# XiaRho/CMDA

Hardware: AMD Instinct MI355X
Metric: training images/sec (512x512 image+event, MiT-B5) (higher is better)
Workload: dtype bf16

## Files before the change

cmda_amd/csrc/gemm.hip:

```cpp
#include "gemm_kernels.h"

namespace {

template <typename T>
int launch_dtype(GemmParams& p, void* stream) {
  const long zb = (long)p.batch * p.batch2;
  auto blocks = [&](int bm, int bn) { return (long)((p.M + bm - 1) / bm) * ((p.N + bn - 1) / bn) * zb; };
  constexpr int BK = 8 * Num<T>::kChunk;
  const int nkt = (p.K + BK - 1) / BK;
  int tile;
  if (p.atomic && p.splits <= 0) {
    tile = 2;
    if (p.M > 64 && p.N > 64) {
      if (sizeof(T) == 2 && p.M >= 256 && p.N >= 256 && p.A.conv != 1 && (blocks(256, 256) >= 32 || (blocks(256, 256) >= 4 && nkt >= 1024)))
        tile = 3;
      else if (blocks(128, 128) >= 64 || (blocks(128, 128) >= 16 && nkt >= 1024)) tile = 0;
      else if (blocks(128, 64) >= 48 && nkt >= 256) tile = 1;
    }
    const long b = tile == 3 ? blocks(256, 256) : tile == 0 ? blocks(128, 128) : tile == 1 ? blocks(128, 64) : blocks(64, 64);
    long s = ((p.B.conv == 1 ? 1024 : 512) + b - 1) / b;
    s = std::min<long>(s, std::max(1, nkt / 8));
    const long out_bytes = (long)p.M * p.N * 4 * zb;
    s = std::min<long>(s, std::max<long>(16, (32L << 20) / std::max<long>(out_bytes, 1)));
    if (tile == 3 && b * s < 256) s = std::min<long>((256 + b - 1) / b, std::max(1, nkt / 8));
    s = std::min<long>(s, 128);
    s = std::min<long>(s, std::max<long>(1, 65535 / std::max<long>(zb, 1)));
    s = std::max<long>(1, s);
    {
      const long slots = 256L * (tile == 3 ? 1 : tile == 0 ? 2 : tile == 1 ? 3 : 4);
      double best = 1e30;
      for (long c = 1; c <= s; ++c) best = std::min(best, (double)((b * c + slots - 1) / slots) / (double)c);
      for (long c = 1; c <= s; ++c)
        if ((double)((b * c + slots - 1) / slots) / (double)c <= best * 1.05) {
          s = c;
          break;
        }
    }
    p.splits = (int)s;
  } else {
    if (p.splits <= 0) p.splits = 1;
    const long sp = p.splits;
    if (sizeof(T) == 2 && p.N >= 256 && p.K >= 256 && (blocks(256, 256) * sp >= 1024 || (blocks(256, 256) * sp >= 200 && p.K >= 2048))) tile = 3;
    else if (sizeof(T) == 2 && (p.N & 255) == 0 && p.K <= 1024 && blocks(256, 256) * sp >= 256 && !p.a_kstrided && !p.b_kstrided && p.A.conv != 1 &&
             p.B.conv != 1 && !p.res && !p.rowscale && p.beta == 0.f && !p.out_f32 && !p.atomic && p.c_patch_ow == 0)
      tile = 3;
    else if (p.N > 64 && (p.N & 127) > 0 && (p.N & 127) <= 64 && blocks(128, 64) * sp >= 2048) tile = 1;
    else if (p.N > 64 && blocks(128, 128) * sp >= 256) tile = 0;
    else if (blocks(128, 64) * sp >= 2048) tile = 1;
    else tile = 2;
    if (tile != 3 && blocks(128, 128) * sp < 1024 && p.M > 64 && p.N > 64) {
      const double nk = (double)nkt;
      const double cost0 = (double)((blocks(128, 128) * sp + 511) / 512) * (4.0 + 0.9 * nk);
      const bool lean = sizeof(T) == 2 && cmda_gemm_lean_ok_(p, 2);
      const double cost1 = (double)((blocks(128, 64) * sp + 767) / 768) * (lean ? 1.5 + 0.45 * nk : 3.0 + 0.75 * nk);
      const double cost2 = (double)((blocks(64, 64) * sp + 1023) / 1024) * (lean ? 1.2 + 0.3 * nk : 2.5 + 0.6 * nk);
      tile = cost0 <= cost1 && cost0 <= cost2 ? 0 : cost1 <= cost2 ? 1 : 2;
    }
  }
  if ((p.tile_hint & 15) >= 1 && (p.tile_hint & 15) <= 4 && p.tile_hint > 0) tile = (p.tile_hint & 15) - 1;
  if constexpr (sizeof(T) == 2) {
    const bool no_glds = p.tile_hint < 0;
    auto dma_ok = [&](const GemmView& v) {
      return v.vec_ok && (v.in_dil <= 1 || (v.conv == 1 && !v.reflect && &v == &p.A && !p.a_kstrided)) && v.R < (1L << 31) && v.Cc < (1L << 31) &&
             (!v.conv || (v.H < 32768 && v.W < 32768)) && (v.conv || (v.ld % 8) == 0) && (v.Cc % 8) == 0 &&
             (v.conv != 2 || ((v.KW * v.C) % 64 == 0 && v.KH == v.stride && v.KW == v.stride && v.pad == 0 && v.dil == 1 &&
                              v.H == v.OH * v.stride && v.W == v.OW * v.stride));
    };
    const bool ac = p.A.conv == 1, bc = p.B.conv == 1, aks = p.a_kstrided != 0, bks = p.b_kstrided != 0;
    const bool kind_ok = (!ac && !bc) || (ac && !bc && !aks && !bks) || (!ac && bc && aks && bks);
    const bool nt_plain = kind_ok && dma_ok(p.A) && dma_ok(p.B);
    if (p.colsum && !(nt_plain && !no_glds && aks)) return CMDA_ERR_UNSUPPORTED;
    if (nt_plain && !no_glds) {
      const bool pp_shape = (p.tile_hint > 0 && (p.tile_hint & 1024)) || (!ac && (p.K <= 1024 || bks));
      if (tile == 3 && pp_shape && !(p.tile_hint > 0 && (p.tile_hint & 512)) && !aks && !bc && !p.atomic && p.splits == 1 && !p.res &&
          !p.rowscale && p.beta == 0.f && !p.out_f32 && p.c_patch_ow == 0 && !p.colsum)
        return cmda_gemm_pp_(p, stream);
      if (tile == 3 && aks && bks && !ac && p.atomic && p.out_f32 && !(p.tile_hint > 0 && (p.tile_hint & 512)))
        return cmda_gemm_wg_(p, stream);
      if (tile == 3) return cmda_gemm_glds_t3_(p, stream);
      if (tile == 0) return cmda_gemm_glds_t0_(p, stream);
      if (!p.colstats && cmda_gemm_lean_ok_(p, tile)) {
        const long tl = tile == 1 ? blocks(128, 64) : blocks(64, 64);
        const int force = p.tile_hint > 0 ? ((p.tile_hint >> 4) & 15) : 0;
        const bool four_stage = force ? force == 4 : (tl <= 256L * (tile == 1 ? 1 : 2) && nkt >= 12);
        return cmda_gemm_lean_(p, tile, four_stage ? 1 : 0, stream);
      }
      if (tile == 1) return cmda_gemm_glds_t1_(p, stream);
      return cmda_gemm_glds_t2_(p, stream);
    }
  }
  if (p.colsum && !(p.dtype == CMDA_F32X3 && cmda_gemm_x3_lean_ok_(p))) return CMDA_ERR_UNSUPPORTED;
  return cmda_gemm_reg_(p, tile, stream);
}

}

extern "C" int cmda_gemm(const cmda_gemm_params_t* pp, void* stream) {
  if (!pp) return CMDA_ERR_SHAPE;
  GemmParams p = *pp;
  if (p.batch2 <= 0) p.batch2 = 1;
  if (p.M <= 0 || p.N <= 0 || p.batch <= 0) return CMDA_OK;
  if (p.K <= 0) return CMDA_ERR_SHAPE;
  if (p.atomic && !p.out_f32) return CMDA_ERR_UNSUPPORTED;
  if (p.splits > 1 && !p.atomic) return CMDA_ERR_UNSUPPORTED;
  if (p.atomic && (p.bias || p.act || p.res || p.rowscale)) return CMDA_ERR_UNSUPPORTED;
  if (p.colstats && (p.atomic || p.splits > 1 || p.act || p.rowscale || p.c_patch_ow > 0 || p.a_kstrided || p.batch != 1 || p.batch2 != 1 || (p.N & 3) ||
                     p.colstats_rows <= 0 || (p.colstats_rows & 255) || p.colsum))
    return CMDA_ERR_UNSUPPORTED;
  if (p.c_patch_ow > 0 && (p.atomic || p.res || p.batch != 1 || p.batch2 != 1 || p.c_patch_kh <= 0 || p.c_patch_kwci <= 0 ||
                           p.N != p.c_patch_kh * p.c_patch_kwci || p.M % p.c_patch_ow != 0 || (p.c_patch_kwci & 3)))
    return CMDA_ERR_UNSUPPORTED;
  if (p.dtype == CMDA_F32 || p.dtype == CMDA_F32X3) return launch_dtype<float>(p, stream);
  if (p.dtype == CMDA_BF16) return launch_dtype<bf16_t>(p, stream);
  return CMDA_ERR_DTYPE;
}

#ifdef CMDA_GEMM_TIMING
#include "gemm_t0.hip"
#include "gemm_t1.hip"
#include "gemm_t2.hip"
#include "gemm_t3.hip"
#include "gemm_reg.hip"
#include "gemm_reg_f32_t0.hip"
#include "gemm_reg_f32_t1.hip"
#include "gemm_reg_f32_t2.hip"
#include "gemm_reg_bf16_t0.hip"
#include "gemm_reg_bf16_t1.hip"
#include "gemm_reg_bf16_t2.hip"
extern "C" int cmda_debug_gemm_stamps(unsigned long long* host_out) {
  return hipMemcpyFromSymbol(host_out, HIP_SYMBOL(g_stamps), sizeof(unsigned long long) * 256 * 8) == hipSuccess ? 0 : -3;
}
#endif
```

cmda_amd/csrc/gemm_kernels.h:

```cpp
#pragma once
#include <cstdlib>
#include <type_traits>
#include "common.h"
#include "../../include/cmda_hip.h"

namespace {

typedef cmda_view_t GemmView;
typedef cmda_gemm_params_t GemmParams;

static __device__ __forceinline__ int reflect_idx(int i, int n) {
  if (i < 0) i = -i;
  if (i >= n) i = 2 * (n - 1) - i;
  return i;
}

static __device__ __forceinline__ long view_offset(const GemmView& v, long r, long c) {
  if (r >= v.R || c >= v.Cc) return -1;
  if (!v.conv) return r * v.ld + c;
  const int ohw = v.OH * v.OW;
  const int b = (int)(r / ohw);
  const int rem = (int)(r - (long)b * ohw);
  const int oh = rem / v.OW;
  const int ow = rem - oh * v.OW;
// ... 824 lines not shown
};

template <bool KS, bool CONV, bool FAST> struct DmaMode { static constexpr int value = !FAST ? 0 : (CONV ? (KS ? 3 : 2) : 1); };

template <int TM, int TN, bool AKS, bool BKS, bool ACONV, bool BCONV, int NW, int NSV, bool FAST = false>
static __device__ __forceinline__ void gemm_glds_body(const GemmParams& p, char* smem, int bt_raw, int ntile_raw, int z_raw, bool xcd_walk) {
  typedef bf16_t T;
  typedef GldsCfg<TM, TN, NW, NSV> Cfg;
  constexpr int WM = Cfg::WM, NTHR = Cfg::NTHR, BM = Cfg::BM, BN = Cfg::BN, BK = Cfg::BK, NS = Cfg::NS;
  constexpr int SZ_A = Cfg::SZ_A, SZ_B = Cfg::SZ_B, PITCH_C = Cfg::PITCH_C, EPI_ROWS = Cfg::EPI_ROWS;
  T* const sAbase = reinterpret_cast<T*>(smem);
  T* const sBbase = sAbase + NS * SZ_A;
  const int tid = threadIdx.x, lane = tid & 63, wid = tid >> 6;
  const int wm = wid >> 1, wn = wid & 1, g = lane >> 4, l15 = lane & 15;
  const int tiles_n = (p.N + BN - 1) / BN;
  const int ntile = ntile_raw;
  int bt = bt_raw;
  if (xcd_walk) {
    const int q = ntile / 8, rr = ntile % 8, xcd = bt % 8, loc = bt / 8;
    bt = (xcd < rr ? xcd * (q + 1) : rr * (q + 1) + (xcd - rr) * q) + loc;
  }
  long mt, nt;
  {
    constexpr int GM = NW == 8 ? 4 : 8;
    const int tiles_m = (int)((p.M + BM - 1) / BM);
    if (tiles_n >= 2 * GM && tiles_m >= GM && !(p.tile_hint > 0 && (p.tile_hint & 256))) {
      const int gsz = GM * tiles_n, gid = bt / gsz, first = gid * GM;
      const int gm = min(tiles_m - first, GM), r = bt - gid * gsz;
      mt = first + r % gm;
      nt = r / gm;
    } else {
      mt = bt / tiles_n;
      nt = bt % tiles_n;
    }
  }
  const long m0 = mt * BM;
  const long n0 = nt * BN;
  const int z = z_raw;
  const int bz = z / p.splits;
  const int split = z - bz * p.splits;
  const int batch = bz / p.batch2, batch2 = bz - batch * p.batch2;
  const int nkt = (p.K + BK - 1) / BK;
  const int kt_per = (nkt + p.splits - 1) / p.splits;
  const int kt0 = split * kt_per;
  const int kt1 = min(nkt, kt0 + kt_per);
  const T* baseA = reinterpret_cast<const T*>(p.A.ptr) + (long)batch * p.A.batch_stride + (long)batch2 * p.A.batch2_stride;
  const T* baseB = reinterpret_cast<const T*>(p.B.ptr) + (long)batch * p.B.batch_stride + (long)batch2 * p.B.batch2_stride;

  CMDA_STAMP(0);
  DmaSrc<AKS, BM, ACONV, NW, 0, 64, DmaMode<AKS, ACONV, FAST>::value> dA;
  DmaSrc<BKS, BN, BCONV, NW, 0, 64, DmaMode<BKS, BCONV, FAST>::value> dB;
  dA.init(p.A, baseA, wid, lane, m0, kt0);
  dB.init(p.B, baseB, wid, lane, n0, kt0);
  auto issue = [&](int stage, int kt) {
    char* la = reinterpret_cast<char*>(sAbase + stage * SZ_A) + wid * dA.J * 1024;
    char* lb = reinterpret_cast<char*>(sBbase + stage * SZ_B) + wid * dB.J * 1024;
    const bool fa = dA.cell_begin(kt, kt0, &p.A), fb = dB.cell_begin(kt, kt0, &p.B);
#pragma unroll
    for (int j = 0; j < dA.J; ++j) glds16(dA.get(p.A, baseA, j, kt, fa), la + j * 1024);
#pragma unroll
    for (int j = 0; j < dB.J; ++j) glds16(dB.get(p.B, baseB, j, kt, fb), lb + j * 1024);
  };

  f32x4 acc[TM][TN];
#pragma unroll
  for (int i = 0; i < TM; ++i)
#pragma unroll
    for (int j = 0; j < TN; ++j) acc[i][j] = f32x4{0.f, 0.f, 0.f, 0.f};

  const bool do_colsum = AKS && p.colsum != nullptr && n0 == 0;
  float bsum = 0.f;
  constexpr int LPT = DmaSrc<AKS, BM, ACONV, NW>::J + DmaSrc<BKS, BN, BCONV, NW>::J;
#pragma unroll
  for (int s = 0; s < NS - 1; ++s)
    if (kt0 + s < kt1) issue(s, kt0 + s);
  CMDA_STAMP(1);
  int st = 0;
  for (int kt = kt0; kt < kt1; ++kt) {
    if (kt + NS - 2 < kt1) pipe_barrier<(NS - 2) * LPT>();
    else pipe_barrier<0>();
    if (kt == kt0) CMDA_STAMP(2);
    {
      int sn = st + NS - 1;
      if (sn >= NS) sn -= NS;
      if (kt + NS - 1 < kt1) issue(sn, kt + NS - 1);
    }
    const T* sA = sAbase + st * SZ_A;
    const T* sB = sBbase + st * SZ_B;
    if constexpr (AKS) {
      if (do_colsum && tid < BM) {
#pragma unroll 8
        for (int k = 0; k < BK; ++k) bsum += bf2f(sA[k * BM + (((tid >> 3) ^ (k & 7)) << 3) + (tid & 7)]);
      }
    }
#pragma unroll
    for (int kk = 0; kk < 2; ++kk) {
      u16x8 fa[TM], fb[TN];
#pragma unroll
      for (int i = 0; i < TM; ++i) {
        const int mr = wm * 16 * TM + i * 16;
        if constexpr (!AKS) {
          const int row = mr + l15;
          fa[i] = *reinterpret_cast<const u16x8*>(&sA[row * BK + (((kk * 4 + g) ^ (row & 7)) << 3)]);
        } else {
          const int q = l15 >> 2, pp = l15 & 3;
          const int k0 = kk * 32 + 8 * g + q, k1 = k0 + 4;
          const int cidx = (mr >> 3) + (pp >> 1), half = (pp & 1) << 2;
          const u16x4 lo = lds_read_tr16(&sA[k0 * BM + ((cidx ^ (k0 & 7)) << 3) + half]);
          const u16x4 hi = lds_read_tr16(&sA[k1 * BM + ((cidx ^ (k1 & 7)) << 3) + half]);
          fa[i] = u16x8{lo[0], lo[1], lo[2], lo[3], hi[0], hi[1], hi[2], hi[3]};
        }
      }
#pragma unroll
      for (int j = 0; j < TN; ++j) {
        const int nr = wn * 16 * TN + j * 16;
        if constexpr (!BKS) {
          const int row = nr + l15;
          fb[j] = *reinterpret_cast<const u16x8*>(&sB[row * BK + (((kk * 4 + g) ^ (row & 7)) << 3)]);
        } else {
          const int q = l15 >> 2, pp = l15 & 3;
          const int k0 = kk * 32 + 8 * g + q, k1 = k0 + 4;
          const int cidx = (nr >> 3) + (pp >> 1), half = (pp & 1) << 2;
          const u16x4 lo = lds_read_tr16(&sB[k0 * BN + ((cidx ^ (k0 & 7)) << 3) + half]);
          const u16x4 hi = lds_read_tr16(&sB[k1 * BN + ((cidx ^ (k1 & 7)) << 3) + half]);
          fb[j] = u16x8{lo[0], lo[1], lo[2], lo[3], hi[0], hi[1], hi[2], hi[3]};
        }
      }
#pragma unroll
      for (int i = 0; i < TM; ++i)
#pragma unroll
        for (int j = 0; j < TN; ++j) acc[i][j] = mfma_bf16_16x16x32(fa[i], fb[j], acc[i][j]);
    }
    if (++st == NS) st = 0;
  }
  CMDA_STAMP(3);
  __syncthreads();

  if (kt0 >= kt1 && p.splits > 1) return;
  if constexpr (AKS) {
    if (do_colsum && tid < BM && m0 + tid < p.M) atomicAdd(p.colsum + m0 + tid, bsum);
  }
  const long cb = (long)batch * p.c_batch_stride + (long)batch2 * p.c_batch2_stride;
  const long rb_off = (long)batch * p.res_batch_stride + (long)batch2 * p.res_batch2_stride;
  if (p.atomic) {
#pragma unroll
    for (int i = 0; i < TM; ++i)
#pragma unroll
      for (int j = 0; j < TN; ++j) {
        const long n = n0 + wn * 16 * TN + j * 16 + l15;
#pragma unroll
        for (int r = 0; r < 4; ++r) {
          const long m = m0 + wm * 16 * TM + i * 16 + 4 * g + r;
          if (m < p.M && n < p.N) atomicAdd(reinterpret_cast<float*>(p.C) + cb + m * p.ldc + atomic_col(p, n), p.alpha * acc[i][j][r]);
        }
      }
    return;
  }
  float* sC = reinterpret_cast<float*>(smem);
  if constexpr (NW == 4) {
#pragma unroll
    for (int i = 0; i < TM; ++i)
#pragma unroll
      for (int j = 0; j < TN; ++j)
#pragma unroll
        for (int r = 0; r < 4; ++r)
          sC[(wm * 16 * TM + i * 16 + 4 * g + r) * PITCH_C + wn * 16 * TN + j * 16 + l15] = acc[i][j][r];
    __syncthreads();
    CMDA_STAMP(4);
    float cs[4] = {0.f, 0.f, 0.f, 0.f}, cq[4] = {0.f, 0.f, 0.f, 0.f};
    epilogue_store<T, BM, BN, PITCH_C, NTHR>(p, sC, m0, n0, cb, rb_off, tid, cs, cq);
    if (p.colstats) {
      __syncthreads();
      colstats_flush<BN, NTHR>(p, sC, m0, n0, tid, cs, cq);
    }
  } else {
    float cs[4] = {0.f, 0.f, 0.f, 0.f}, cq[4] = {0.f, 0.f, 0.f, 0.f};
    for (int wr = 0; wr < WM; ++wr) {
      if (wm == wr) {
#pragma unroll
        for (int i = 0; i < TM; ++i)
#pragma unroll
          for (int j = 0; j < TN; ++j)
#pragma unroll
            for (int r = 0; r < 4; ++r)
              sC[(i * 16 + 4 * g + r) * PITCH_C + wn * 16 * TN + j * 16 + l15] = acc[i][j][r];
      }
      __syncthreads();
      if (m0 + wr * EPI_ROWS < p.M)
        epilogue_store<T, EPI_ROWS, BN, PITCH_C, NTHR>(p, sC, m0 + wr * EPI_ROWS, n0, cb, rb_off, tid, cs, cq);
      __syncthreads();
    }
    if (p.colstats) colstats_flush<BN, NTHR>(p, sC, m0, n0, tid, cs, cq);
    CMDA_STAMP(4);
  }
  CMDA_STAMP(5);
}

template <int TM, int TN, bool AKS, bool BKS, bool ACONV, bool BCONV, int NW = 4, int NSV = 0, bool FAST = false>
__global__ __launch_bounds__(64 * NW, (GldsCfg<TM, TN, NW, NSV>::MIN_WAVES)) void gemm_glds_kernel(GemmParams p) {
  __shared__ __attribute__((aligned(1024))) char smem[GldsCfg<TM, TN, NW, NSV>::LDS_BYTES];
  gemm_glds_body<TM, TN, AKS, BKS, ACONV, BCONV, NW, NSV, FAST>(p, smem, blockIdx.x, gridDim.x, blockIdx.z, true);
}

template <int TM, int TN, bool AKS, bool BKS, bool ACONV, bool BCONV, int NW = 4, int NSV = 0, bool FAST = false>
__global__ __launch_bounds__(64 * NW, (GldsCfg<TM, TN, NW, NSV>::MIN_WAVES)) void gemm_glds_grouped_kernel(const GemmParams* __restrict__ tab,
                                                                                                            const int* __restrict__ blk) {
  __shared__ __attribute__((aligned(1024))) char smem[GldsCfg<TM, TN, NW, NSV>::LDS_BYTES];
#ifndef CMDA_EMU
  const int prob = __builtin_amdgcn_readfirstlane(blk[2 * blockIdx.x]), loc = __builtin_amdgcn_readfirstlane(blk[2 * blockIdx.x + 1]);
#else
  const int prob = blk[2 * blockIdx.x], loc = blk[2 * blockIdx.x + 1];
#endif
  if (prob < 0) return;
  const GemmParams& p = tab[prob];
  constexpr int BM = GldsCfg<TM, TN, NW, NSV>::BM, BN = GldsCfg<TM, TN, NW, NSV>::BN;
  const int ntile = (int)((p.M + BM - 1) / BM) * ((p.N + BN - 1) / BN);
  const int z = loc / ntile;
  gemm_glds_body<TM, TN, AKS, BKS, ACONV, BCONV, NW, NSV, FAST>(p, smem, loc - z * ntile, ntile, z, false);
}

template <int TM, int TN, int NW, int NSV, bool AKS, bool BKS, bool ACONV, bool BCONV>
int launch_glds_mode(const GemmParams& p, const dim3& grid, void* stream) {
  constexpr int BM = 16 * TM * (NW / 2), BN = 32 * TN;
  const dim3 blk(64 * NW);
  typedef DmaSrc<AKS, BM, ACONV, NW, 0, 64, DmaMode<AKS, ACONV, true>::value> FA;
  typedef DmaSrc<BKS, BN, BCONV, NW, 0, 64, DmaMode<BKS, BCONV, true>::value> FB;
  const bool fast = FA::mode_ok(p.A, FA::MODE) && FB::mode_ok(p.B, FB::MODE) && (FA::MODE != 0 || FB::MODE != 0) &&
                    !(p.tile_hint > 0 && (p.tile_hint & 2048));
  if (fast) CMDA_LAUNCH((gemm_glds_kernel<TM, TN, AKS, BKS, ACONV, BCONV, NW, NSV, true>), grid, blk, 0, stream, p);
  else CMDA_LAUNCH((gemm_glds_kernel<TM, TN, AKS, BKS, ACONV, BCONV, NW, NSV, false>), grid, blk, 0, stream, p);
  CMDA_CHECK_LAUNCH();
}

template <int TM, int TN, int NW, int NSV>
int launch_glds_ns(const GemmParams& p, const dim3& grid, void* stream) {
  const bool aks = p.a_kstrided != 0, bks = p.b_kstrided != 0, ac = p.A.conv == 1, bc = p.B.conv == 1;
  if (!aks && !bks && !ac && !bc) return launch_glds_mode<TM, TN, NW, NSV, false, false, false, false>(p, grid, stream);
  if (!aks && bks && !ac && !bc) return launch_glds_mode<TM, TN, NW, NSV, false, true, false, false>(p, grid, stream);
  if (aks && bks && !ac && !bc) return launch_glds_mode<TM, TN, NW, NSV, true, true, false, false>(p, grid, stream);
  if (aks && !bks && !ac && !bc) return launch_glds_mode<TM, TN, NW, NSV, true, false, false, false>(p, grid, stream);
  if (!aks && !bks && ac && !bc) return launch_glds_mode<TM, TN, NW, NSV, false, false, true, false>(p, grid, stream);
  if (aks && bks && !ac && bc) return launch_glds_mode<TM, TN, NW, NSV, true, true, false, true>(p, grid, stream);
  return CMDA_ERR_UNSUPPORTED;
}

template <int TM, int TN, int NW = 4>
int launch_glds(const GemmParams& p, void* stream) {
  constexpr int BM = 16 * TM * (NW / 2), BN = 32 * TN;
  const long tiles = (long)((p.M + BM - 1) / BM) * ((p.N + BN - 1) / BN);
  const long zz = (long)p.batch * p.batch2 * p.splits;
  if (tiles > 0x7fffffffL || zz > 65535) return CMDA_ERR_SHAPE;
  dim3 grid((unsigned)tiles, 1, (unsigned)zz);
  if constexpr (NW == 4) {
    constexpr long kStage = (long)(BM + BN) * 128;
    const long resident = 256L * (4 * kStage <= 65536 ? 2 : 1);
    const long nkt = ((long)p.K + 63) / 64 / (p.splits > 0 ? p.splits : 1);
    const int force = p.tile_hint > 0 ? ((p.tile_hint >> 4) & 15) : 0;
    if (force) return force == 4 ? launch_glds_ns<TM, TN, NW, 4>(p, grid, stream) : launch_glds_ns<TM, TN, NW, 0>(p, grid, stream);
    const int min_nkt = (p.tile_hint > 0 && (p.tile_hint >> 12)) ? (p.tile_hint >> 12) : 12;
    if (tiles * zz <= resident && nkt >= min_nkt) return launch_glds_ns<TM, TN, NW, 4>(p, grid, stream);
  }
  return launch_glds_ns<TM, TN, NW, 0>(p, grid, stream);
}

template <int TM, int TN, int NW = 4>
int launch_glds_grouped(const GemmParams* tab, const void* blk, int nblocks, int bconv, void* stream) {
  if (nblocks <= 0) return CMDA_OK;
  const dim3 grid((unsigned)nblocks), blkdim(64 * NW);
  const int* b = reinterpret_cast<const int*>(blk);
  if (bconv == 2) CMDA_LAUNCH((gemm_glds_grouped_kernel<TM, TN, true, true, false, true, NW, 0, false>), grid, blkdim, 0, stream, tab, b);
  else if (bconv == 1) CMDA_LAUNCH((gemm_glds_grouped_kernel<TM, TN, true, true, false, false, NW, 0, false>), grid, blkdim, 0, stream, tab, b);
  else CMDA_LAUNCH((gemm_glds_grouped_kernel<TM, TN, true, true, false, false, NW, 0, true>), grid, blkdim, 0, stream, tab, b);
  CMDA_CHECK_LAUNCH();
}

template <typename T, int TM, int TN>
int launch_tile(const GemmParams& p, void* stream) {
  constexpr int BM = 32 * TM, BN = 32 * TN;
  const long tiles = (long)((p.M + BM - 1) / BM) * ((p.N + BN - 1) / BN);
  if (tiles > 0x7fffffffL || (long)p.batch * p.batch2 * p.splits > 65535) return CMDA_ERR_SHAPE;
  dim3 grid((unsigned)tiles, 1, (unsigned)(p.batch * p.batch2 * p.splits));
  const bool aks = p.a_kstrided != 0, bks = p.b_kstrided != 0;
  if (!aks && !bks) CMDA_LAUNCH((gemm_kernel<T, TM, TN, false, false>), grid, dim3(256), 0, stream, p);
  else if (!aks && bks) CMDA_LAUNCH((gemm_kernel<T, TM, TN, false, true>), grid, dim3(256), 0, stream, p);
  else if (aks && bks) CMDA_LAUNCH((gemm_kernel<T, TM, TN, true, true>), grid, dim3(256), 0, stream, p);
  else CMDA_LAUNCH((gemm_kernel<T, TM, TN, true, false>), grid, dim3(256), 0, stream, p);
  CMDA_CHECK_LAUNCH();
}

}

int cmda_gemm_glds_t0_(const cmda_gemm_params_t& p, void* stream);
int cmda_gemm_glds_t1_(const cmda_gemm_params_t& p, void* stream);
int cmda_gemm_glds_t2_(const cmda_gemm_params_t& p, void* stream);
int cmda_gemm_glds_t3_(const cmda_gemm_params_t& p, void* stream);
bool cmda_gemm_lean_ok_(const cmda_gemm_params_t& p, int tile);
int cmda_gemm_lean_(const cmda_gemm_params_t& p, int tile, int four_stage, void* stream);
int cmda_gemm_grouped_t2_(const cmda_gemm_params_t* tab, const void* blk, int nblocks, int bconv, void* stream);
int cmda_gemm_grouped_t0_(const cmda_gemm_params_t* tab, const void* blk, int nblocks, int bconv, void* stream);
int cmda_gemm_grouped_t1_(const cmda_gemm_params_t* tab, const void* blk, int nblocks, int bconv, void* stream);
int cmda_gemm_grouped_t3_(const cmda_gemm_params_t* tab, const void* blk, int nblocks, int bconv, void* stream);
int cmda_gemm_wg_grouped_(const cmda_gemm_params_t* tab, const void* blk, int nblocks, int bconv, void* stream);
int cmda_gemm_wg_(const cmda_gemm_params_t& p, void* stream);
int cmda_gemm_pp_(const cmda_gemm_params_t& p, void* stream);
int cmda_gemm_reg_(const cmda_gemm_params_t& p, int tile, void* stream);
int cmda_gemm_x3_(const cmda_gemm_params_t& p, int tile, void* stream);
bool cmda_gemm_x3_lean_ok_(const cmda_gemm_params_t& p);
int cmda_gemm_x3_lean_(const cmda_gemm_params_t& p, void* stream);
int cmda_gemm_x3_lean_grouped_(const cmda_gemm_params_t* tab, const void* blk, int nblocks, void* stream);
int cmda_gemm_reg_f32_t0_(const cmda_gemm_params_t& p, void* stream);
int cmda_gemm_reg_f32_t1_(const cmda_gemm_params_t& p, void* stream);
int cmda_gemm_reg_f32_t2_(const cmda_gemm_params_t& p, void* stream);
int cmda_gemm_reg_bf16_t0_(const cmda_gemm_params_t& p, void* stream);
int cmda_gemm_reg_bf16_t1_(const cmda_gemm_params_t& p, void* stream);
int cmda_gemm_reg_bf16_t2_(const cmda_gemm_params_t& p, void* stream);
```

cmda_amd/csrc/gemm_pp.hip:

```cpp
#include "gemm_kernels.h"

namespace {

typedef __attribute__((ext_vector_type(16))) float f32x16;

#ifndef CMDA_EMU
static __device__ __forceinline__ f32x16 mfma_bf16_32x32x16(u16x8 a, u16x8 b, f32x16 c) {
  return __builtin_amdgcn_mfma_f32_32x32x16_bf16(__builtin_bit_cast(bfx8, a), __builtin_bit_cast(bfx8, b), c, 0, 0, 0);
}
static __device__ __forceinline__ void raw_barrier() { __builtin_amdgcn_s_barrier(); }
static __device__ __forceinline__ void sched_fence() { __builtin_amdgcn_sched_barrier(0); }
static __device__ __forceinline__ void prio(int hi) {
  if (hi) __builtin_amdgcn_s_setprio(1);
  else __builtin_amdgcn_s_setprio(0);
}
static __device__ __forceinline__ void wait_lds() { asm volatile("s_waitcnt lgkmcnt(0)" ::: "memory"); }
static __device__ __forceinline__ void wait_dma_lds() { asm volatile("s_waitcnt vmcnt(0) lgkmcnt(0)" ::: "memory"); }
#else
static inline f32x16 mfma_bf16_32x32x16(u16x8 a, u16x8 b, f32x16 c) {
  auto& w = emu::my_wave();
  const int l = emu::my_lane();
  for (int j = 0; j < 8; ++j) { w.fa[l][j] = bf2f(a[j]); w.fb[l][j] = bf2f(b[j]); }
  emu::wave_barrier();
  const int col = l & 31, h = l >> 5;
  f32x16 d = c;
  for (int r = 0; r < 16; ++r) {
    const int row = (r & 3) + 8 * (r >> 2) + 4 * h;
    float acc = d[r];
    for (int hh = 0; hh < 2; ++hh)
      for (int j = 0; j < 8; ++j) acc = fmaf(w.fa[32 * hh + row][j], w.fb[32 * hh + col][j], acc);
    d[r] = acc;
  }
  emu::wave_barrier();
  return d;
}
static inline void raw_barrier() { __syncthreads(); }
static inline void sched_fence() {}
static inline void prio(int) {}
static inline void wait_lds() {}
static inline void wait_dma_lds() { emu::wave_barrier(); }
#endif

#ifdef CMDA_PP_TIMING
__device__ unsigned long long g_pp_stamps[2 * 4 * 4 * 4];
#define PP_STAMP(i) do { if (lane == 0 && (wid & 3) == 0 && blockIdx.x == 7 && kt >= 8 && kt < 12) \
    g_pp_stamps[((grp * 4 + (kt - 8)) * 4 + q) * 4 + (i)] = __builtin_amdgcn_s_memtime(); } while (0)
#else
#define PP_STAMP(i) do { } while (0)
#endif

constexpr int PP_BM = 256, PP_BN = 256, PP_BK = 64, PP_NW = 8;
constexpr int PP_SZ = PP_BM * PP_BK;
constexpr int PP_PITCH_C = PP_BN + 8;
constexpr size_t PP_LDS = (size_t)PP_BM * PP_PITCH_C * 2;

template <int ACT>
static __device__ __forceinline__ float pp_act(float x) {
  if (ACT == 1) return fmaxf(x, 0.f);
  if (ACT == 2) return gelu_erf(x);
  if (ACT == 3) return tanhf(x);
  return x;
}

template <bool BKS, bool ACONV, bool FAST = false>
__global__ __launch_bounds__(512, 1) void gemm_pp_kernel(GemmParams p) {
  typedef bf16_t T;
  __shared__ __attribute__((aligned(1024))) char smem[PP_LDS];
  T* const sAbase = reinterpret_cast<T*>(smem);
  T* const sBbase = sAbase + 2 * PP_SZ;

  const int tid = threadIdx.x, lane = tid & 63;
#ifndef CMDA_EMU
  const int wid = __builtin_amdgcn_readfirstlane(tid >> 6);
#else
  const int wid = tid >> 6;
#endif
  const int grp = wid >> 2, wc = wid & 3;
  const int l31 = lane & 31, h = lane >> 5;

  const int tiles_n = (p.N + PP_BN - 1) / PP_BN;
  const int ntile = gridDim.x;
  int bt = blockIdx.x;
  {
    const int q = ntile / 8, rr = ntile % 8, xcd = bt % 8, loc = bt / 8;
    bt = (xcd < rr ? xcd * (q + 1) : rr * (q + 1) + (xcd - rr) * q) + loc;
  }
  long mt, nt;
  {
    constexpr int GM = 4;
    const int tiles_m = (int)((p.M + PP_BM - 1) / PP_BM);
    if (tiles_n >= 2 * GM && tiles_m >= GM) {
      const int gsz = GM * tiles_n, gid = bt / gsz, first = gid * GM;
      const int gm = min(tiles_m - first, GM), r = bt - gid * gsz;
      mt = first + r % gm;
      nt = r / gm;
    } else {
      mt = bt / tiles_n;
      nt = bt % tiles_n;
    }
  }
  const long m0 = mt * PP_BM, n0 = nt * PP_BN;
  const int z = blockIdx.z;
  const int batch = z / p.batch2, batch2 = z - batch * p.batch2;
  const int nkt = (p.K + PP_BK - 1) / PP_BK;
  const T* baseA = reinterpret_cast<const T*>(p.A.ptr) + (long)batch * p.A.batch_stride + (long)batch2 * p.A.batch2_stride;
  const T* baseB = reinterpret_cast<const T*>(p.B.ptr) + (long)batch * p.B.batch_stride + (long)batch2 * p.B.batch2_stride;

  DmaSrc<false, PP_BM, ACONV, PP_NW, 1, 64, DmaMode<false, ACONV, FAST>::value> dA;
  DmaSrc<BKS, PP_BN, false, PP_NW, 1, 64, DmaMode<BKS, false, FAST>::value> dB;
  dA.init(p.A, baseA, wid, lane, m0, 0);
  dB.init(p.B, baseB, wid, lane, n0, 0);
  bool cellA = false;
  auto piece = [&](int stage, int kt, int i) {
    if (i == 0) cellA = dA.cell_begin(kt, 0);
    if (i < 4) glds16(dA.get(p.A, baseA, i, kt, cellA), reinterpret_cast<char*>(sAbase + stage * PP_SZ) + (wid * 4 + i) * 1024);
    else glds16(dB.get(p.B, baseB, i - 4, kt, false), reinterpret_cast<char*>(sBbase + stage * PP_SZ) + (wid * 4 + (i - 4)) * 1024);
  };

  f32x16 acc[4][2];
#pragma unroll
  for (int i = 0; i < 4; ++i)
#pragma unroll
    for (int j = 0; j < 2; ++j)
#pragma unroll
      for (int r = 0; r < 16; ++r) acc[i][j][r] = 0.f;

  auto load_a = [&](const T* sA, int mh, u16x8 (&fa)[2][4]) {
#pragma unroll
    for (int i = 0; i < 2; ++i) {
      const int row = grp * 128 + (mh * 2 + i) * 32 + l31;
#pragma unroll
      for (int s = 0; s < 4; ++s) fa[i][s] = *reinterpret_cast<const u16x8*>(&sA[row * PP_BK + (((2 * s + h) ^ ((row >> 1) & 7)) << 3)]);
    }
  };
  auto load_b = [&](const T* sB, int nh, u16x8 (&fb)[4]) {
    if constexpr (!BKS) {
      const int row = wc * 64 + nh * 32 + l31;
#pragma unroll
      for (int s = 0; s < 4; ++s) fb[s] = *reinterpret_cast<const u16x8*>(&sB[row * PP_BK + (((2 * s + h) ^ ((row >> 1) & 7)) << 3)]);
    } else {
      const int gi = lane >> 4, li = lane & 15, q = li >> 2, pp = li & 3;
      const int colbase = wc * 64 + nh * 32 + 16 * (gi & 1);
      const int cidx = (colbase >> 3) + (pp >> 1), half = (pp & 1) << 2;
#pragma unroll
      for (int s = 0; s < 4; ++s) {
        const int k0 = 16 * s + 8 * (gi >> 1) + q, k1 = k0 + 4;
        const u16x4 lo = lds_read_tr16(&sB[k0 * PP_BN + ((cidx ^ (k0 & 7)) << 3) + half]);
        const u16x4 hi = lds_read_tr16(&sB[k1 * PP_BN + ((cidx ^ (k1 & 7)) << 3) + half]);
        fb[s] = u16x8{lo[0], lo[1], lo[2], lo[3], hi[0], hi[1], hi[2], hi[3]};
      }
    }
  };

#pragma unroll
  for (int i = 0; i < 8; ++i) piece(0, 0, i);
  wait_dma_lds();
  raw_barrier();
  if (grp == 1) raw_barrier();

  u16x8 fa[2][4], fb[2][4];
  for (int kt = 0; kt < nkt; ++kt) {
    const int st = kt & 1;
    const T* sA = sAbase + st * PP_SZ;
    const T* sB = sBbase + st * PP_SZ;
    const bool more = kt + 1 < nkt;
#pragma unroll
    for (int q = 0; q < 4; ++q) {
      const int mh = q >> 1, nh = (q == 1 || q == 2) ? 1 : 0;
      PP_STAMP(0);
      if (q == 0 || q == 2) load_a(sA, mh, fa);
      if (q < 2) load_b(sB, nh, fb[nh]);
      if (more) {
        if (q == 0) { piece(st ^ 1, kt + 1, 0); piece(st ^ 1, kt + 1, 4); }
        if (q == 1) { piece(st ^ 1, kt + 1, 1); piece(st ^ 1, kt + 1, 2); piece(st ^ 1, kt + 1, 5); piece(st ^ 1, kt + 1, 6); }
        if (q == 2) { piece(st ^ 1, kt + 1, 3); piece(st ^ 1, kt + 1, 7); }
      }
      if (q == 3 && grp == 1) wait_dma_lds();
      if (q == 3 && grp == 0) wait_lds();
      sched_fence();
      raw_barrier();
      wait_lds();
      PP_STAMP(1);
      sched_fence();
      prio(1);
#pragma unroll
      for (int s = 0; s < 4; ++s)
#pragma unroll
        for (int i = 0; i < 2; ++i) acc[mh * 2 + i][nh] = mfma_bf16_32x32x16(fb[nh][s], fa[i][s], acc[mh * 2 + i][nh]);
      prio(0);
      PP_STAMP(2);
      if (q == 3 && grp == 0) wait_dma_lds();
      sched_fence();
      raw_barrier();
      PP_STAMP(3);
    }
  }
  if (grp == 0) raw_barrier();
  __syncthreads();

  T* sC = reinterpret_cast<T*>(smem);
  const float alpha = p.alpha;
  const int act = p.act;
#pragma unroll
  for (int j = 0; j < 2; ++j)
#pragma unroll
    for (int rg = 0; rg < 4; ++rg) {
      const int nl = wc * 64 + j * 32 + 8 * rg + 4 * h;
      float bv[4] = {0.f, 0.f, 0.f, 0.f};
      if (p.bias) {
#pragma unroll
        for (int e = 0; e < 4; ++e)
          if (n0 + nl + e < p.N) bv[e] = p.bias[n0 + nl + e];
      }
#pragma unroll
      for (int i = 0; i < 4; ++i) {
        const int ml = grp * 128 + i * 32 + l31;
        float v[4];
#pragma unroll
        for (int e = 0; e < 4; ++e) v[e] = alpha * acc[i][j][rg * 4 + e] + bv[e];
        if (act == 1) {
#pragma unroll
          for (int e = 0; e < 4; ++e) v[e] = pp_act<1>(v[e]);
        } else if (act == 2) {
#pragma unroll
          for (int e = 0; e < 4; ++e) v[e] = pp_act<2>(v[e]);
        } else if (act == 3) {
#pragma unroll
          for (int e = 0; e < 4; ++e) v[e] = pp_act<3>(v[e]);
        }
        st4(&sC[ml * PP_PITCH_C + nl], v);
      }
    }
  __syncthreads();
  const long cb = (long)batch * p.c_batch_stride + (long)batch2 * p.c_batch2_stride;
  T* C = reinterpret_cast<T*>(p.C) + cb;
  const bool vec = p.c_vec_ok != 0 && (p.ldc & 7) == 0 && ((reinterpret_cast<uintptr_t>(C) & 15) == 0);
  const bool stats = p.colstats != nullptr;
  float cs[8] = {0.f, 0.f, 0.f, 0.f, 0.f, 0.f, 0.f, 0.f}, cq[8] = {0.f, 0.f, 0.f, 0.f, 0.f, 0.f, 0.f, 0.f};
#pragma unroll 4
  for (int it = 0; it < (PP_BM * PP_BN / 8) / 512; ++it) {
    const int idx = it * 512 + tid;
    const int row = idx >> 5, ch = idx & 31;
    const long m = m0 + row, n = n0 + ch * 8;
    if (m >= p.M || n >= p.N) continue;
    const uint4 val = *reinterpret_cast<const uint4*>(&sC[row * PP_PITCH_C + ch * 8]);
    if (stats) {
      T tv[8];
      __builtin_memcpy(tv, &val, 16);
#pragma unroll
      for (int e = 0; e < 8; ++e) {
        const float f = bf2f(tv[e]);
        cs[e] += f;
        cq[e] += f * f;
      }
    }
    if (vec && n + 8 <= p.N) {
      *reinterpret_cast<uint4*>(&C[m * p.ldc + n]) = val;
    } else {
      T tmp[8];
      __builtin_memcpy(tmp, &val, 16);
#pragma unroll
      for (int e = 0; e < 8; ++e)
        if (n + e < p.N) C[m * p.ldc + n + e] = tmp[e];
    }
  }
  if (stats) {
#pragma unroll
    for (int e = 0; e < 8; ++e) {
      cs[e] += __shfl_xor(cs[e], 32, 64);
      cq[e] += __shfl_xor(cq[e], 32, 64);
    }
    __syncthreads();
    float* scr = reinterpret_cast<float*>(smem);
    const int wv = tid >> 6, ln = tid & 63;
    if (ln < 32) {
#pragma unroll
      for (int e = 0; e < 8; ++e) {
        scr[wv * 2 * PP_BN + ln * 8 + e] = cs[e];
        scr[wv * 2 * PP_BN + PP_BN + ln * 8 + e] = cq[e];
      }
    }
    __syncthreads();
    static_assert(2 * PP_BN == 512, "one thread per (statistic, column)");
    const int col = tid & (PP_BN - 1);
    if (n0 + col < p.N) {
      float t = 0.f;
#pragma unroll
      for (int w = 0; w < 8; ++w) t += scr[w * 2 * PP_BN + tid];
      const long gidx = (unsigned)m0 / (unsigned)p.colstats_rows;
      const unsigned slot = (unsigned)(m0 >> 6) & (CMDA_BN_SLOTS - 1);
      atomicAdd(p.colstats + (gidx * (CMDA_BN_SLOTS + 1) + slot) * 2 * (long)p.N + (tid < PP_BN ? 0 : p.N) + n0 + col, t);
    }
  }
}

}

#ifdef CMDA_PP_TIMING
extern "C" int cmda_debug_pp_stamps(unsigned long long* host_out) {
  return hipMemcpyFromSymbol(host_out, HIP_SYMBOL(g_pp_stamps), sizeof(unsigned long long) * 128) == hipSuccess ? 0 : -3;
}
#endif

int cmda_gemm_pp_(const cmda_gemm_params_t& p, void* stream) {
  const long tiles = (long)((p.M + PP_BM - 1) / PP_BM) * ((p.N + PP_BN - 1) / PP_BN);
  const long zz = (long)p.batch * p.batch2;
  if (tiles > 0x7fffffffL || zz > 65535) return CMDA_ERR_SHAPE;
  const dim3 grid((unsigned)tiles, 1, (unsigned)zz), blk(512);
  const bool bks = p.b_kstrided != 0, ac = p.A.conv == 1;
  if (p.a_kstrided || p.B.conv == 1) return CMDA_ERR_UNSUPPORTED;
  const bool nofast = p.tile_hint > 0 && (p.tile_hint & 2048);
  typedef DmaSrc<false, PP_BM, false, PP_NW, 1, 64, 1> FA;
  typedef DmaSrc<false, PP_BM, true, PP_NW, 1, 64, 2> FAC;
  typedef DmaSrc<false, PP_BN, false, PP_NW, 1, 64, 1> FB;
  typedef DmaSrc<true, PP_BN, false, PP_NW, 1, 64, 1> FBK;
  if (!bks && !ac) {
    if (!nofast && FA::mode_ok(p.A, 1) && FB::mode_ok(p.B, 1)) CMDA_LAUNCH((gemm_pp_kernel<false, false, true>), grid, blk, 0, stream, p);
    else CMDA_LAUNCH((gemm_pp_kernel<false, false, false>), grid, blk, 0, stream, p);
  } else if (!bks && ac) {
    if (!nofast && FAC::mode_ok(p.A, 2) && FB::mode_ok(p.B, 1)) CMDA_LAUNCH((gemm_pp_kernel<false, true, true>), grid, blk, 0, stream, p);
    else CMDA_LAUNCH((gemm_pp_kernel<false, true, false>), grid, blk, 0, stream, p);
  } else if (bks && !ac) {
    if (!nofast && FA::mode_ok(p.A, 1) && FBK::mode_ok(p.B, 1)) CMDA_LAUNCH((gemm_pp_kernel<true, false, true>), grid, blk, 0, stream, p);
    else CMDA_LAUNCH((gemm_pp_kernel<true, false, false>), grid, blk, 0, stream, p);
  }
  else return CMDA_ERR_UNSUPPORTED;
  CMDA_CHECK_LAUNCH();
}
```

Measured before the change: 39.26.

## Split PP GEMM DMA into half-tiles with two-ahead prefetch and register column stats

For the non-K-strided path, the PP GEMM kernel now issues global-to-LDS DMA in half-tile pieces across two descriptor sets per operand. Loads run up to two K-steps ahead, and a partial vmcnt wait keeps later loads in flight instead of draining all of them each step. Column statistics are also accumulated in fp32 from the accumulators in registers, reduced with lane shuffles, and written to LDS. This replaces the re-read of bf16 values during store, but only when the shape selector marks the call as having used the PP path for a non-default reason. The changes add register pressure (64 extra floats) and rely on hand-counted waitcnt values, which risks races if the instruction counts differ.

```diff
diff --git a/cmda_amd/csrc/gemm.hip b/cmda_amd/csrc/gemm.hip
--- a/cmda_amd/csrc/gemm.hip
+++ b/cmda_amd/csrc/gemm.hip
@@ -71,10 +71,11 @@
     const bool nt_plain = kind_ok && dma_ok(p.A) && dma_ok(p.B);
     if (p.colsum && !(nt_plain && !no_glds && aks)) return CMDA_ERR_UNSUPPORTED;
     if (nt_plain && !no_glds) {
-      const bool pp_shape = (p.tile_hint > 0 && (p.tile_hint & 1024)) || (!ac && (p.K <= 1024 || bks));
+      const bool pp_before = !ac && (p.K <= 1024 || bks);
+      const bool pp_shape = (p.tile_hint > 0 && (p.tile_hint & 1024)) || pp_before;
       if (tile == 3 && pp_shape && !(p.tile_hint > 0 && (p.tile_hint & 512)) && !aks && !bc && !p.atomic && p.splits == 1 && !p.res &&
           !p.rowscale && p.beta == 0.f && !p.out_f32 && p.c_patch_ow == 0 && !p.colsum)
-        return cmda_gemm_pp_(p, stream);
+        return cmda_gemm_pp_(p, stream, pp_before ? 0 : 1);
       if (tile == 3 && aks && bks && !ac && p.atomic && p.out_f32 && !(p.tile_hint > 0 && (p.tile_hint & 512)))
         return cmda_gemm_wg_(p, stream);
       if (tile == 3) return cmda_gemm_glds_t3_(p, stream);
diff --git a/cmda_amd/csrc/gemm_kernels.h b/cmda_amd/csrc/gemm_kernels.h
--- a/cmda_amd/csrc/gemm_kernels.h
+++ b/cmda_amd/csrc/gemm_kernels.h
@@ -1150,7 +1150,7 @@
 int cmda_gemm_grouped_t3_(const cmda_gemm_params_t* tab, const void* blk, int nblocks, int bconv, void* stream);
 int cmda_gemm_wg_grouped_(const cmda_gemm_params_t* tab, const void* blk, int nblocks, int bconv, void* stream);
 int cmda_gemm_wg_(const cmda_gemm_params_t& p, void* stream);
-int cmda_gemm_pp_(const cmda_gemm_params_t& p, void* stream);
+int cmda_gemm_pp_(const cmda_gemm_params_t& p, void* stream, int stats_f32);
 int cmda_gemm_reg_(const cmda_gemm_params_t& p, int tile, void* stream);
 int cmda_gemm_x3_(const cmda_gemm_params_t& p, int tile, void* stream);
 bool cmda_gemm_x3_lean_ok_(const cmda_gemm_params_t& p);
diff --git a/cmda_amd/csrc/gemm_pp.hip b/cmda_amd/csrc/gemm_pp.hip
--- a/cmda_amd/csrc/gemm_pp.hip
+++ b/cmda_amd/csrc/gemm_pp.hip
@@ -16,6 +16,8 @@
 }
 static __device__ __forceinline__ void wait_lds() { asm volatile("s_waitcnt lgkmcnt(0)" ::: "memory"); }
 static __device__ __forceinline__ void wait_dma_lds() { asm volatile("s_waitcnt vmcnt(0) lgkmcnt(0)" ::: "memory"); }
+static __device__ __forceinline__ void wait_dma_keep3() { asm volatile("s_waitcnt vmcnt(6)" ::: "memory"); }
+static __device__ __forceinline__ void wait_dma_all() { asm volatile("s_waitcnt vmcnt(0)" ::: "memory"); }
 #else
 static inline f32x16 mfma_bf16_32x32x16(u16x8 a, u16x8 b, f32x16 c) {
   auto& w = emu::my_wave();
@@ -39,6 +41,8 @@
 static inline void prio(int) {}
 static inline void wait_lds() {}
 static inline void wait_dma_lds() { emu::wave_barrier(); }
+static inline void wait_dma_keep3() { emu::wave_barrier(); }
+static inline void wait_dma_all() { emu::wave_barrier(); }
 #endif
 
 #ifdef CMDA_PP_TIMING
@@ -63,7 +67,7 @@
 }
 
 template <bool BKS, bool ACONV, bool FAST = false>
-__global__ __launch_bounds__(512, 1) void gemm_pp_kernel(GemmParams p) {
+__global__ __launch_bounds__(512, 1) void gemm_pp_kernel(GemmParams p, int stats_f32) {
   typedef bf16_t T;
   __shared__ __attribute__((aligned(1024))) char smem[PP_LDS];
   T* const sAbase = reinterpret_cast<T*>(smem);
@@ -106,17 +110,6 @@
   const T* baseA = reinterpret_cast<const T*>(p.A.ptr) + (long)batch * p.A.batch_stride + (long)batch2 * p.A.batch2_stride;
   const T* baseB = reinterpret_cast<const T*>(p.B.ptr) + (long)batch * p.B.batch_stride + (long)batch2 * p.B.batch2_stride;
 
-  DmaSrc<false, PP_BM, ACONV, PP_NW, 1, 64, DmaMode<false, ACONV, FAST>::value> dA;
-  DmaSrc<BKS, PP_BN, false, PP_NW, 1, 64, DmaMode<BKS, false, FAST>::value> dB;
-  dA.init(p.A, baseA, wid, lane, m0, 0);
-  dB.init(p.B, baseB, wid, lane, n0, 0);
-  bool cellA = false;
-  auto piece = [&](int stage, int kt, int i) {
-    if (i == 0) cellA = dA.cell_begin(kt, 0);
-    if (i < 4) glds16(dA.get(p.A, baseA, i, kt, cellA), reinterpret_cast<char*>(sAbase + stage * PP_SZ) + (wid * 4 + i) * 1024);
-    else glds16(dB.get(p.B, baseB, i - 4, kt, false), reinterpret_cast<char*>(sBbase + stage * PP_SZ) + (wid * 4 + (i - 4)) * 1024);
-  };
-
   f32x16 acc[4][2];
 #pragma unroll
   for (int i = 0; i < 4; ++i)
@@ -152,9 +145,57 @@
     }
   };
 
-#pragma unroll
-  for (int i = 0; i < 8; ++i) piece(0, 0, i);
-  wait_dma_lds();
+  typedef DmaSrc<false, PP_BM, ACONV, 2 * PP_NW, 1, 64, DmaMode<false, ACONV, FAST>::value> SrcA;
+  typedef DmaSrc<false, PP_BN, false, 2 * PP_NW, 1, 64, DmaMode<false, false, FAST>::value> SrcB;
+  typedef DmaSrc<false, PP_BM, ACONV, PP_NW, 1, 64, DmaMode<false, ACONV, FAST>::value> SrcAK;
+  typedef DmaSrc<true, PP_BN, false, PP_NW, 1, 64, DmaMode<true, false, FAST>::value> SrcBK;
+  static_assert(SrcA::J == 2 && SrcB::J == 2 && SrcAK::J == 4 && SrcBK::J == 4, "DMA instructions per wave and half-tile / stage");
+  const int wa = (wid >> 2) * 8 + (wid & 3), wb = (wid >> 1) * 4 + (wid & 1);
+  SrcA dA0, dA1;
+  SrcB dB0, dB1;
+  SrcAK dAK;
+  SrcBK dBK;
+  if constexpr (!BKS) {
+    dA0.init(p.A, baseA, wa, lane, m0, 0);
+    dA1.init(p.A, baseA, wa + 4, lane, m0, 0);
+    dB0.init(p.B, baseB, wb, lane, n0, 0);
+    dB1.init(p.B, baseB, wb + 2, lane, n0, 0);
+  } else {
+    dAK.init(p.A, baseA, wid, lane, m0, 0);
+    dBK.init(p.B, baseB, wid, lane, n0, 0);
+  }
+  auto half = [&](auto& d, const GemmView& v, const T* base, char* dst, int kt) {
+    const bool first = d.cell_begin(kt, 0, &v);
+    glds16(d.get(v, base, 0, kt, first), dst);
+    glds16(d.get(v, base, 1, kt, first), dst + 1024);
+  };
+  auto stA = [&](int stage, int hh) { return reinterpret_cast<char*>(sAbase + stage * PP_SZ) + (wa + 4 * hh) * 2048; };
+  auto stB = [&](int stage, int hh) { return reinterpret_cast<char*>(sBbase + stage * PP_SZ) + (wb + 2 * hh) * 2048; };
+  bool cellA = false;
+  auto pieceK = [&](int stage, int kt, int i) {
+    if (i == 0) cellA = dAK.cell_begin(kt, 0);
+    if (i < 4) glds16(dAK.get(p.A, baseA, i, kt, cellA), reinterpret_cast<char*>(sAbase + stage * PP_SZ) + (wid * 4 + i) * 1024);
+    else glds16(dBK.get(p.B, baseB, i - 4, kt, false), reinterpret_cast<char*>(sBbase + stage * PP_SZ) + (wid * 4 + (i - 4)) * 1024);
+  };
+
+  if constexpr (!BKS) {
+    half(dA0, p.A, baseA, stA(0, 0), 0);
+    half(dB0, p.B, baseB, stB(0, 0), 0);
+    half(dB1, p.B, baseB, stB(0, 1), 0);
+    half(dA1, p.A, baseA, stA(0, 1), 0);
+    if (nkt > 1) {
+      half(dA0, p.A, baseA, stA(1, 0), 1);
+      half(dB0, p.B, baseB, stB(1, 0), 1);
+      half(dB1, p.B, baseB, stB(1, 1), 1);
+      wait_dma_keep3();
+    } else {
+      wait_dma_all();
+    }
+  } else {
+#pragma unroll
+    for (int i = 0; i < 8; ++i) pieceK(0, 0, i);
+    wait_dma_lds();
+  }
   raw_barrier();
   if (grp == 1) raw_barrier();
 
@@ -163,19 +204,29 @@
     const int st = kt & 1;
     const T* sA = sAbase + st * PP_SZ;
     const T* sB = sBbase + st * PP_SZ;
-    const bool more = kt + 1 < nkt;
 #pragma unroll
     for (int q = 0; q < 4; ++q) {
       const int mh = q >> 1, nh = (q == 1 || q == 2) ? 1 : 0;
       PP_STAMP(0);
       if (q == 0 || q == 2) load_a(sA, mh, fa);
       if (q < 2) load_b(sB, nh, fb[nh]);
-      if (more) {
-        if (q == 0) { piece(st ^ 1, kt + 1, 0); piece(st ^ 1, kt + 1, 4); }
-        if (q == 1) { piece(st ^ 1, kt + 1, 1); piece(st ^ 1, kt + 1, 2); piece(st ^ 1, kt + 1, 5); piece(st ^ 1, kt + 1, 6); }
-        if (q == 2) { piece(st ^ 1, kt + 1, 3); piece(st ^ 1, kt + 1, 7); }
-      }
-      if (q == 3 && grp == 1) wait_dma_lds();
+      if constexpr (!BKS) {
+        if (q == 0 && kt + 1 < nkt) half(dA1, p.A, baseA, stA(st ^ 1, 1), kt + 1);
+        if (q == 2 && kt + 2 < nkt) {
+          half(dA0, p.A, baseA, stA(st, 0), kt + 2);
+          half(dB0, p.B, baseB, stB(st, 0), kt + 2);
+        }
+        if (q == 3 && kt + 2 < nkt) half(dB1, p.B, baseB, stB(st, 1), kt + 2);
+      } else if (kt + 1 < nkt) {
+        if (q == 0) { pieceK(st ^ 1, kt + 1, 0); pieceK(st ^ 1, kt + 1, 4); }
+        if (q == 1) { pieceK(st ^ 1, kt + 1, 1); pieceK(st ^ 1, kt + 1, 2); pieceK(st ^ 1, kt + 1, 5); pieceK(st ^ 1, kt + 1, 6); }
+        if (q == 2) { pieceK(st ^ 1, kt + 1, 3); pieceK(st ^ 1, kt + 1, 7); }
+      }
+      if (q == 3 && grp == 1) {
+        if constexpr (BKS) wait_dma_lds();
+        else if (kt + 2 < nkt) wait_dma_keep3();
+        else wait_dma_all();
+      }
       if (q == 3 && grp == 0) wait_lds();
       sched_fence();
       raw_barrier();
@@ -189,7 +240,11 @@
         for (int i = 0; i < 2; ++i) acc[mh * 2 + i][nh] = mfma_bf16_32x32x16(fb[nh][s], fa[i][s], acc[mh * 2 + i][nh]);
       prio(0);
       PP_STAMP(2);
-      if (q == 3 && grp == 0) wait_dma_lds();
+      if (q == 3 && grp == 0) {
+        if constexpr (BKS) wait_dma_lds();
+        else if (kt + 2 < nkt) wait_dma_keep3();
+        else wait_dma_all();
+      }
       sched_fence();
       raw_barrier();
       PP_STAMP(3);
@@ -201,6 +256,10 @@
   T* sC = reinterpret_cast<T*>(smem);
   const float alpha = p.alpha;
   const int act = p.act;
+  const bool stats = p.colstats != nullptr, s32 = !BKS && stats && stats_f32 != 0;
+  float sv[64];
+#pragma unroll
+  for (int c = 0; c < 64; ++c) sv[c] = 0.f;
 #pragma unroll
   for (int j = 0; j < 2; ++j)
 #pragma unroll
@@ -228,14 +287,34 @@
 #pragma unroll
           for (int e = 0; e < 4; ++e) v[e] = pp_act<3>(v[e]);
         }
+        if (s32 && m0 + ml < p.M) {
+#pragma unroll
+          for (int e = 0; e < 4; ++e) {
+            sv[j * 16 + rg * 4 + e] += v[e];
+            sv[32 + j * 16 + rg * 4 + e] += v[e] * v[e];
+          }
+        }
         st4(&sC[ml * PP_PITCH_C + nl], v);
       }
     }
+  if (s32) {
+#pragma unroll
+    for (int step = 0; step < 5; ++step) {
+      const int nv = 64 >> step, bit = 4 - step;
+      const bool up = (l31 >> bit) & 1;
+#pragma unroll
+      for (int i = 0; i < nv / 2; ++i) {
+        const float give = up ? sv[i] : sv[i + nv / 2];
+        const float keep = up ? sv[i + nv / 2] : sv[i];
+        sv[i] = keep + __shfl_xor(give, 1 << bit, 64);
+      }
+    }
+  }
   __syncthreads();
   const long cb = (long)batch * p.c_batch_stride + (long)batch2 * p.c_batch2_stride;
   T* C = reinterpret_cast<T*>(p.C) + cb;
   const bool vec = p.c_vec_ok != 0 && (p.ldc & 7) == 0 && ((reinterpret_cast<uintptr_t>(C) & 15) == 0);
-  const bool stats = p.colstats != nullptr;
+  const bool s16 = stats && !s32;
   float cs[8] = {0.f, 0.f, 0.f, 0.f, 0.f, 0.f, 0.f, 0.f}, cq[8] = {0.f, 0.f, 0.f, 0.f, 0.f, 0.f, 0.f, 0.f};
 #pragma unroll 4
   for (int it = 0; it < (PP_BM * PP_BN / 8) / 512; ++it) {
@@ -244,7 +323,7 @@
     const long m = m0 + row, n = n0 + ch * 8;
     if (m >= p.M || n >= p.N) continue;
     const uint4 val = *reinterpret_cast<const uint4*>(&sC[row * PP_PITCH_C + ch * 8]);
-    if (stats) {
+    if (s16) {
       T tv[8];
       __builtin_memcpy(tv, &val, 16);
 #pragma unroll
@@ -265,19 +344,27 @@
     }
   }
   if (stats) {
-#pragma unroll
-    for (int e = 0; e < 8; ++e) {
-      cs[e] += __shfl_xor(cs[e], 32, 64);
-      cq[e] += __shfl_xor(cq[e], 32, 64);
-    }
-    __syncthreads();
     float* scr = reinterpret_cast<float*>(smem);
-    const int wv = tid >> 6, ln = tid & 63;
-    if (ln < 32) {
+    if (s32) {
+      __syncthreads();
+      const int cl = wc * 64 + 32 * ((l31 >> 3) & 1) + 8 * ((l31 >> 1) & 3) + 4 * h + 2 * (l31 & 1);
+      float* d = scr + (grp * 2 + (l31 >> 4)) * PP_BN + cl;
+      d[0] = sv[0];
+      d[1] = sv[1];
+    } else {
 #pragma unroll
       for (int e = 0; e < 8; ++e) {
-        scr[wv * 2 * PP_BN + ln * 8 + e] = cs[e];
-        scr[wv * 2 * PP_BN + PP_BN + ln * 8 + e] = cq[e];
+        cs[e] += __shfl_xor(cs[e], 32, 64);
+        cq[e] += __shfl_xor(cq[e], 32, 64);
+      }
+      __syncthreads();
+      const int wv = tid >> 6, ln = tid & 63;
+      if (ln < 32) {
+#pragma unroll
+        for (int e = 0; e < 8; ++e) {
+          scr[wv * 2 * PP_BN + ln * 8 + e] = cs[e];
+          scr[wv * 2 * PP_BN + PP_BN + ln * 8 + e] = cq[e];
+        }
       }
     }
     __syncthreads();
@@ -285,8 +372,12 @@
     const int col = tid & (PP_BN - 1);
     if (n0 + col < p.N) {
       float t = 0.f;
-#pragma unroll
-      for (int w = 0; w < 8; ++w) t += scr[w * 2 * PP_BN + tid];
+      if (s32) {
+        t = scr[tid] + scr[2 * PP_BN + tid];
+      } else {
+#pragma unroll
+        for (int w = 0; w < 8; ++w) t += scr[w * 2 * PP_BN + tid];
+      }
       const long gidx = (unsigned)m0 / (unsigned)p.colstats_rows;
       const unsigned slot = (unsigned)(m0 >> 6) & (CMDA_BN_SLOTS - 1);
       atomicAdd(p.colstats + (gidx * (CMDA_BN_SLOTS + 1) + slot) * 2 * (long)p.N + (tid < PP_BN ? 0 : p.N) + n0 + col, t);
@@ -302,7 +393,7 @@
 }
 #endif
 
-int cmda_gemm_pp_(const cmda_gemm_params_t& p, void* stream) {
+int cmda_gemm_pp_(const cmda_gemm_params_t& p, void* stream, int stats_f32) {
   const long tiles = (long)((p.M + PP_BM - 1) / PP_BM) * ((p.N + PP_BN - 1) / PP_BN);
   const long zz = (long)p.batch * p.batch2;
   if (tiles > 0x7fffffffL || zz > 65535) return CMDA_ERR_SHAPE;
@@ -315,14 +406,14 @@
   typedef DmaSrc<false, PP_BN, false, PP_NW, 1, 64, 1> FB;
   typedef DmaSrc<true, PP_BN, false, PP_NW, 1, 64, 1> FBK;
   if (!bks && !ac) {
-    if (!nofast && FA::mode_ok(p.A, 1) && FB::mode_ok(p.B, 1)) CMDA_LAUNCH((gemm_pp_kernel<false, false, true>), grid, blk, 0, stream, p);
-    else CMDA_LAUNCH((gemm_pp_kernel<false, false, false>), grid, blk, 0, stream, p);
+    if (!nofast && FA::mode_ok(p.A, 1) && FB::mode_ok(p.B, 1)) CMDA_LAUNCH((gemm_pp_kernel<false, false, true>), grid, blk, 0, stream, p, stats_f32);
+    else CMDA_LAUNCH((gemm_pp_kernel<false, false, false>), grid, blk, 0, stream, p, stats_f32);
   } else if (!bks && ac) {
-    if (!nofast && FAC::mode_ok(p.A, 2) && FB::mode_ok(p.B, 1)) CMDA_LAUNCH((gemm_pp_kernel<false, true, true>), grid, blk, 0, stream, p);
-    else CMDA_LAUNCH((gemm_pp_kernel<false, true, false>), grid, blk, 0, stream, p);
+    if (!nofast && FAC::mode_ok(p.A, 2) && FB::mode_ok(p.B, 1)) CMDA_LAUNCH((gemm_pp_kernel<false, true, true>), grid, blk, 0, stream, p, stats_f32);
+    else CMDA_LAUNCH((gemm_pp_kernel<false, true, false>), grid, blk, 0, stream, p, stats_f32);
   } else if (bks && !ac) {
-    if (!nofast && FA::mode_ok(p.A, 1) && FBK::mode_ok(p.B, 1)) CMDA_LAUNCH((gemm_pp_kernel<true, false, true>), grid, blk, 0, stream, p);
-    else CMDA_LAUNCH((gemm_pp_kernel<true, false, false>), grid, blk, 0, stream, p);
+    if (!nofast && FA::mode_ok(p.A, 1) && FBK::mode_ok(p.B, 1)) CMDA_LAUNCH((gemm_pp_kernel<true, false, true>), grid, blk, 0, stream, p, stats_f32);
+    else CMDA_LAUNCH((gemm_pp_kernel<true, false, false>), grid, blk, 0, stream, p, stats_f32);
   }
   else return CMDA_ERR_UNSUPPORTED;
   CMDA_CHECK_LAUNCH();
```

Measured after the change: 39.23, median of 2. No clear change (-0.1%).
